# jiaxi98/cnf_ot

Measured on AMD Instinct MI355X. Metric: MC samples/sec through flow fwd+log|detJ| at dim=2, batch=65536, higher is better.
Workload: dtype f32; 1 GPU; configs[1]: OT free dim=2, batch=65536, sample_and_log_prob (RQS fwd + log|detJ|), L=2 H=16 M=2 K=5, params N(0,0.20^2) seed 42; ONE STEP = one evaluator-shaped pass of 10000 time-slices x 65536 samples (cnf_ot/utils.py:311-340), each slice its own condition t, one cnf_sample_logprob call per rank; batch=65536, dim=2, parallelism=slice-shard x1 (contiguous blocks of the step's slices; no collective)

## Files before the change

### cnf_ot_amd/csrc/cnf_common.h

```cpp
#pragma once
#include <mutex>
#include <map>
#include <tuple>
#include <unordered_map>
#include <vector>

#include "cnf_device.h"
#include "cnf_terms.h"
#include "../../include/cnf_ot_amd.h"

namespace cnf {

constexpr int TILE = 256;

struct ModelArgs {
  const float* prep;
  const float* wq;
  int64_t per_layer;
  int64_t per_layer_q;
  int32_t D, L, M;
  SplineConsts sc;
  SplineConstsT<double> scd;
  const double* tabd;
  const double* e2tab;
};

template <class R> __device__ __forceinline__ const SplineConstsT<R>& sc_of(const ModelArgs& a);
template <> __device__ __forceinline__ const SplineConstsT<float>& sc_of<float>(const ModelArgs& a) { return a.sc; }
template <> __device__ __forceinline__ const SplineConstsT<double>& sc_of<double>(const ModelArgs& a) { return a.scd; }
template <class R> __device__ __forceinline__ const R* table_of(const ModelArgs& a);
template <> __device__ __forceinline__ const float* table_of<float>(const ModelArgs& a) { return a.prep; }
template <> __device__ __forceinline__ const double* table_of<double>(const ModelArgs& a) { return a.tabd; }

}

struct CnfModel {
  CnfConfig cfg;
  cnf::SplineConsts sc;
  cnf::SplineConstsT<double> scd;
  int64_t tabd_off;
  int64_t e2_off;
  int precise;
  float* prep;
  int64_t n_params;
  int64_t per_layer;
  int device;
  int num_cus;
  int fast_math;
  int force_spl;
  int use_mfma;
  uint32_t div_magic;
  int64_t per_layer_q;
  int64_t mfma_off;
  int params_set;
  float* grad_slabs;
  int64_t grad_max_blocks;
  int use_pwl;
  int use_dpar;
  float* pwl_stats;
  struct PwlWorkspace { float* tables; int64_t sets; uint32_t epoch; std::vector<float*> retired; };
  std::mutex pwl_mu;
  std::unordered_map<void*, PwlWorkspace> pwl_ws;
  hipEvent_t prep_event;
  void* prep_stream;
  int last_path;
  struct ProfRec { hipEvent_t e0, e1, e2; int64_t samples; int path; };
  int profiling;
  std::vector<ProfRec> prof;
};

enum CnfPath {
  CNF_PATH_NONE = 0,
  CNF_PATH_MLP1 = 1,
  CNF_PATH_MLP2 = 2,
  CNF_PATH_MFMA = 3,
  CNF_PATH_TABLES = 4,
  CNF_PATH_LOSS_MLP = 5,
  CNF_PATH_LOSS_TABLES = 6,
  CNF_PATH_F64 = 7,
  CNF_PATH_DPAR = 9,
  CNF_PATH_DETECT = 8,
  CNF_PATH_FIELDS = 10,
};

static inline bool pwl_network(const CnfConfig& g) {
  return g.dim == 2 && g.hidden_size == 16 && g.num_bins == 5 && g.mlp_num_layers == 2 && !g.periodized;
}
static inline bool pwl_backward_network(const CnfConfig& g) { return pwl_network(g) && g.num_layers <= 4; }
static inline bool pwl_config_ok(const CnfModel* m) { return m->use_pwl && m->fast_math && pwl_network(m->cfg); }
static inline bool pwl_backward_ok(const CnfModel* m) {
  return pwl_config_ok(m) && pwl_backward_network(m->cfg) && m->pwl_stats != nullptr;
}
constexpr int64_t PWL_MIN_SLICE = 8192, PWL_MIN_POINTS = 262144;
static inline bool pwl_term_on_tables(const CnfModel* m, int64_t slice_len, int64_t n_points, bool with_grad) {
  if (with_grad ? !pwl_backward_ok(m) : !pwl_config_ok(m)) return false;
  return m->use_pwl != 1 || (slice_len >= PWL_MIN_SLICE && n_points >= PWL_MIN_POINTS);
}

#ifdef CNF_MINIMAL_CONFIGS
#define CNF_KERNEL_CONFIGS(X) X(16, 5)
#else
#define CNF_KERNEL_CONFIGS(X) \
  X(8, 5) X(16, 4) X(16, 5) X(16, 8) X(16, 10) X(32, 5) X(32, 8) X(64, 5)
#endif

template <class K>
static inline bool ensure_lds(K kernel, size_t bytes) {
  if (bytes > 160 * 1024) return false;
  if (bytes <= 64 * 1024) return true;
  static std::mutex mu;
  static std::map<std::pair<const void*, int>, bool> done;
  int dev = 0;
  if (hipGetDevice(&dev) != hipSuccess) return false;
// ... 85 lines not shown
```

### cnf_ot_amd/csrc/cnf_flow.hip

```cpp
#include "cnf_common.h"
#include <cstdlib>
#include "cnf_pwl_build.h"

#include <math.h>
#include <new>
#include <stdlib.h>
#include <string.h>

namespace cnf {


enum CMode { C_SINGLE = 0, C_PER_SAMPLE = 1, C_TILE_UNIFORM = 2, C_GENERIC = 3 };
enum AuxMode { AUX_LOGDET = 0, AUX_LOGPROB = 1 };


template <class R> struct FlowArgsT {
  ModelArgs m;
  const R* in;
  const R* c;
  R* out;
  R* aux;
  int64_t B;
  int64_t c_block;
  int32_t c_mode, aux_mode;
// ... 1218 lines not shown
  if (!config_valid(cfg)) return CNF_ERR_INVALID;
  if (!cnf_config_supported(cfg)) return CNF_ERR_UNSUPPORTED;
  CnfModel* m = new (std::nothrow) CnfModel();
  if (!m) return CNF_ERR_NOMEM;
  m->cfg = *cfg;
  const int K = cfg->num_bins, P = 3 * K + 1;
  m->n_params = cnf_param_count(cfg);
  m->per_layer = 0;
  for (int d = 1; d < cfg->dim; ++d)
    m->per_layer += cond_floats_p(d, cfg->hidden_size, cfg->mlp_num_layers, P, cfg->periodized != 0);
  m->sc.lo = cfg->range_min; m->sc.hi = cfg->range_max;
  m->sc.min_bin = cfg->min_bin_size; m->sc.min_slope = cfg->min_knot_slope;
  m->sc.span_eff = (float)(((double)cfg->range_max - (double)cfg->range_min) - (double)K * (double)cfg->min_bin_size);
  m->sc.sp_offset = (float)log(exp(1.0 - (double)cfg->min_knot_slope) - 1.0);
  m->fast_math = 1;
  if (hipGetDevice(&m->device) != hipSuccess) { delete m; return CNF_ERR_HIP; }
  hipDeviceProp_t prop;
  if (hipGetDeviceProperties(&prop, m->device) != hipSuccess) { delete m; return CNF_ERR_HIP; }
  m->num_cus = prop.multiProcessorCount;
  m->use_mfma = 2;
  m->use_pwl = 1;
  m->use_dpar = 1;
  m->div_magic = cfg->dim == 1 ? 0u : (uint32_t)((((uint64_t)1 << 32) + (uint64_t)cfg->dim - 1) / (uint64_t)cfg->dim);
  m->per_layer_q = 0; m->mfma_off = 0;
  size_t q_floats = 0;
  if (cfg->hidden_size == 16 && P == 16 && cfg->dim > 1 && !cfg->periodized) {
    for (int d = 1; d < cfg->dim; ++d) m->per_layer_q += cond_floats_mfma(d, cfg->mlp_num_layers);
    m->mfma_off = (hdr_floats(K) + (m->n_params - P) + 3) & ~(int64_t)3;
    q_floats = (size_t)m->per_layer_q * cfg->num_layers;
  }
  m->tabd_off = (hdr_floats(K) + (m->n_params - P) + 4 + (int64_t)q_floats + 1) & ~(int64_t)1;
  m->e2_off = m->tabd_off + 2 * hdr_floats(K);
  m->precise = 1;
  const size_t bytes = (size_t)(m->e2_off + 2 * cnf::EXP2_N) * sizeof(float) + 64;
  m->scd.lo = (double)cfg->range_min; m->scd.hi = (double)cfg->range_max;
  m->scd.min_bin = (double)cfg->min_bin_size; m->scd.min_slope = (double)cfg->min_knot_slope;
  m->scd.span_eff = (m->scd.hi - m->scd.lo) - (double)K * m->scd.min_bin;
  m->scd.sp_offset = log(exp(1.0 - m->scd.min_slope) - 1.0);
  if (hipMalloc((void**)&m->prep, bytes) != hipSuccess) { delete m; return CNF_ERR_NOMEM; }
  {
    double e2[cnf::EXP2_N];
    for (int i = 0; i < cnf::EXP2_N; ++i) e2[i] = exp2(-(double)i / (double)cnf::EXP2_STEPS);
    if (hipMemcpy(m->prep + m->e2_off, e2, sizeof(e2), hipMemcpyHostToDevice) != hipSuccess) {
      (void)hipFree(m->prep); delete m; return CNF_ERR_HIP;
    }
  }
  if (hipEventCreateWithFlags(&m->prep_event, hipEventDisableTiming) != hipSuccess) {
    (void)hipFree(m->prep); delete m; return CNF_ERR_HIP;
  }
  *out = m;
  return CNF_OK;
}

static void prof_clear(CnfModel* m) {
  for (auto& r : m->prof) {
    if (r.e0) (void)hipEventDestroy(r.e0);
    if (r.e1) (void)hipEventDestroy(r.e1);
    if (r.e2) (void)hipEventDestroy(r.e2);
  }
  m->prof.clear();
}

extern "C" void cnf_model_destroy(CnfModel* m) {
  if (!m) return;
  if (m->prep) (void)hipFree(m->prep);
  if (m->grad_slabs) (void)hipFree(m->grad_slabs);
  if (m->pwl_stats) (void)hipFree(m->pwl_stats);
  for (auto& kv : m->pwl_ws) {
    if (kv.second.tables) (void)hipFree(kv.second.tables);
    for (float* p : kv.second.retired) (void)hipFree(p);
  }
  if (m->prep_event) (void)hipEventDestroy(m->prep_event);
  prof_clear(m);
  delete m;
}

extern "C" int cnf_model_last_path(const CnfModel* m) { return m ? m->last_path : CNF_ERR_INVALID; }

extern "C" int cnf_model_set_profiling(CnfModel* m, int on) {
  if (!m) return CNF_ERR_INVALID;
  m->profiling = on ? 1 : 0;
  if (!on) prof_clear(m);
  return CNF_OK;
}

extern "C" int cnf_model_read_profile(CnfModel* m, double* flow_ms, double* build_ms, int64_t* launches,
                                      int64_t* samples) {
  if (!m) return CNF_ERR_INVALID;
  double f = 0.0, b = 0.0;
  int64_t n = 0, smp = 0;
  for (auto& r : m->prof) {
    if (hipEventSynchronize(r.e2) != hipSuccess) return CNF_ERR_HIP;
    float ms = 0.f;
    if (r.e0) { if (hipEventElapsedTime(&ms, r.e0, r.e1) != hipSuccess) return CNF_ERR_HIP; b += ms; }
    if (hipEventElapsedTime(&ms, r.e1, r.e2) != hipSuccess) return CNF_ERR_HIP;
    f += ms; ++n; smp += r.samples;
  }
  prof_clear(m);
  if (flow_ms) *flow_ms = f;
  if (build_ms) *build_ms = b;
  if (launches) *launches = n;
  if (samples) *samples = smp;
  return CNF_OK;
}

struct ProfScope {
  CnfModel* m; hipStream_t s; CnfModel::ProfRec r; bool on;
  ProfScope(CnfModel* m_, hipStream_t s_, bool with_build, int64_t samples, int path) : m(m_), s(s_), on(false) {
    r.e0 = r.e1 = r.e2 = nullptr; r.samples = samples; r.path = path;
    if (!m->profiling || m->prof.size() >= 4096) return;
    if (hipEventCreate(&r.e1) != hipSuccess || hipEventCreate(&r.e2) != hipSuccess) return;
    if (with_build) { if (hipEventCreate(&r.e0) != hipSuccess) return; (void)hipEventRecord(r.e0, s); }
    else (void)hipEventRecord(r.e1, s);
    on = true;
  }
  void built() { if (on && r.e0) (void)hipEventRecord(r.e1, s); }
  void done() { if (on) { (void)hipEventRecord(r.e2, s); m->prof.push_back(r); on = false; } }
};

extern "C" int cnf_model_set_fast_math(CnfModel* m, int on) {
  if (!m) return CNF_ERR_INVALID;
  m->fast_math = on ? 1 : 0;
  return CNF_OK;
// ... 116 lines not shown
    if (!a.gate) m->last_path = CNF_PATH_MLP1;
#define X(HH, KK)                                                                             \
    if (m->cfg.hidden_size == HH && m->cfg.num_bins == KK) {                                  \
      CNF_LAUNCH((flow_kernel<HH, KK, TO_BASE, true, float, false, false, true>), grid1, lds1, stream, a);  \
      return hipGetLastError() == hipSuccess ? CNF_OK : CNF_ERR_HIP;                          \
    }
    CNF_KERNEL_CONFIGS(X)
#undef X
    return CNF_ERR_UNSUPPORTED;
  }
  const bool precise = PR && m->precise;
  const size_t lds = (size_t)(hdr_floats(m->cfg.num_bins) + 2 * a.m.D * ts) * sizeof(float) +
                     (precise ? precise_lds_bytes(m->cfg.num_bins) + sizeof(float) * a.m.D * ts : 0);
  const bool small = a.B <= (int64_t)m->num_cus * 4 * 64 * CNF_MFMA_SMALL_WAVES;
  if (m->fast_math && (m->use_mfma == 1 || (m->use_mfma == 2 && small)) && m->mfma_off > 0 &&
      m->cfg.hidden_size == 16 && m->cfg.num_bins == 5) {
    if (!a.gate) m->last_path = CNF_PATH_MFMA;
    ProfScope ps(m, stream, false, a.B, CNF_PATH_MFMA);
    const bool d2 = m->cfg.dim == 2 && spl == 1;
    if (precise) {
      if (spl == 2) CNF_LAUNCH((flow_kernel<16, 5, TO_BASE, true, v2f, true, PR>), grid, lds, stream, a);
      else if (d2) CNF_LAUNCH((flow_kernel<16, 5, TO_BASE, true, float, true, PR, false, 2>), grid, lds, stream, a);
      else CNF_LAUNCH((flow_kernel<16, 5, TO_BASE, true, float, true, PR>), grid, lds, stream, a);
    } else {
      if (spl == 2) CNF_LAUNCH((flow_kernel<16, 5, TO_BASE, true, v2f, true>), grid, lds, stream, a);
      else if (d2) CNF_LAUNCH((flow_kernel<16, 5, TO_BASE, true, float, true, false, false, 2>), grid, lds, stream, a);
      else CNF_LAUNCH((flow_kernel<16, 5, TO_BASE, true, float, true>), grid, lds, stream, a);
    }
    ps.done();
    return hipGetLastError() == hipSuccess ? CNF_OK : CNF_ERR_HIP;
  }
  if (!a.gate) m->last_path = spl == 2 ? CNF_PATH_MLP2 : CNF_PATH_MLP1;
  ProfScope ps(m, stream, false, a.B, spl == 2 ? CNF_PATH_MLP2 : CNF_PATH_MLP1);
#define X(HH, KK)                                                                             \
  if (m->cfg.hidden_size == HH && m->cfg.num_bins == KK) {                                    \
    if (precise) {                                                                            \
      if (!m->fast_math) CNF_LAUNCH((flow_kernel<HH, KK, TO_BASE, false, float, false, PR>), grid, lds, stream, a);  \
      else if (spl == 2) CNF_LAUNCH((flow_kernel<HH, KK, TO_BASE, true, v2f, false, PR>), grid, lds, stream, a);     \
      else CNF_LAUNCH((flow_kernel<HH, KK, TO_BASE, true, float, false, PR>), grid, lds, stream, a);                 \
    } else {                                                                                  \
      if (!m->fast_math) CNF_LAUNCH((flow_kernel<HH, KK, TO_BASE, false, float>), grid, lds, stream, a);      \
      else if (spl == 2) CNF_LAUNCH((flow_kernel<HH, KK, TO_BASE, true, v2f>), grid, lds, stream, a);         \
      else CNF_LAUNCH((flow_kernel<HH, KK, TO_BASE, true, float>), grid, lds, stream, a);                     \
    }                                                                                         \
    ps.done();                                                                                \
    return hipGetLastError() == hipSuccess ? CNF_OK : CNF_ERR_HIP;                            \
  }
  CNF_KERNEL_CONFIGS(X)
#undef X
  return CNF_ERR_UNSUPPORTED;
}

static void pwl_workspace(CnfModel* m, hipStream_t stream, float** tables, int64_t* sets, uint32_t** flag = nullptr,
                          uint32_t* epoch = nullptr) {
  std::lock_guard<std::mutex> lock(m->pwl_mu);
  auto it = m->pwl_ws.find((void*)stream);
  if (it == m->pwl_ws.end()) { *tables = nullptr; *sets = 0; return; }
  *tables = it->second.tables; *sets = it->second.sets;
  if (flag) { *flag = reinterpret_cast<uint32_t*>(it->second.tables + it->second.sets * m->cfg.num_layers * (int64_t)cnf::PWL_TBL);
              *epoch = ++it->second.epoch; }
}

extern "C" int64_t cnf_model_table_bytes(const CnfModel* m) {
  return m ? (int64_t)sizeof(float) * m->cfg.num_layers * cnf::PWL_TBL : 0;
}

extern "C" int cnf_model_reserve(CnfModel* m, void* stream, int64_t n_sets) {
  if (!m || n_sets < 0) return CNF_ERR_INVALID;
  std::lock_guard<std::mutex> lock(m->pwl_mu);
  CnfModel::PwlWorkspace& ws = m->pwl_ws[stream];
  if (ws.sets >= n_sets && n_sets > 0) return CNF_OK;
  if (ws.tables && n_sets > 0) {
    ws.retired.push_back(ws.tables);
    ws.tables = nullptr; ws.sets = 0;
  }
  if (n_sets == 0) {
    if (hipStreamSynchronize((hipStream_t)stream) != hipSuccess) return CNF_ERR_HIP;
    if (ws.tables) (void)hipFree(ws.tables);
    for (float* p : ws.retired) (void)hipFree(p);
    m->pwl_ws.erase(stream);
    return CNF_OK;
  }
  if (hipMalloc((void**)&ws.tables, (size_t)cnf_model_table_bytes(m) * (size_t)n_sets + 64) != hipSuccess) {
    ws.tables = nullptr; ws.sets = 0;
    return CNF_ERR_NOMEM;
  }
  if (hipMemset(reinterpret_cast<char*>(ws.tables) + (size_t)cnf_model_table_bytes(m) * (size_t)n_sets, 0, 64) != hipSuccess) {
    (void)hipFree(ws.tables); ws.tables = nullptr; ws.sets = 0;
    return CNF_ERR_HIP;
  }
  ws.sets = n_sets; ws.epoch = 0;
  return CNF_OK;
}

extern "C" int64_t cnf_model_reserved(CnfModel* m, void* stream) {
  if (!m) return CNF_ERR_INVALID;
  float* t; int64_t sets;
  pwl_workspace(m, (hipStream_t)stream, &t, &sets);
  return sets;
}

static const int64_t PWL_MAX_SLICES = 2048;

static_assert(cnf::PWL_H == 16, "pwl_network (cnf_common.h) states the tables' network");

extern "C" int cnf_model_has_tables(const CnfModel* m) { return m && pwl_network(m->cfg) ? 1 : 0; }

extern "C" int cnf_model_term_on_tables(const CnfModel* m, int64_t slice_len, int64_t n_points, int with_grad) {
  return m && pwl_term_on_tables(m, slice_len, n_points, with_grad != 0) ? 1 : 0;
}

struct NoiseSrc { uint64_t seed; int64_t first_sample, slice_stride; };

static int run_flow_pwl(CnfModel* m, bool to_base, const float* in, const float* c, int64_t c_block,
                        float* out, float* aux, int aux_mode, int64_t B, hipStream_t stream,
                        bool detect = false, const uint32_t** gate = nullptr, uint32_t* gate_epoch = nullptr,
                        const NoiseSrc* noise = nullptr, const float* built = nullptr, bool in_shared = false) {
  if (!pwl_config_ok(m)) return CNF_ERR_UNSUPPORTED;
  const int L = m->cfg.num_layers;
  const bool precise = to_base && m->precise;
  auto lds_for = [&](int lrows) {
    return (size_t)(((cnf::hdr_floats(5) + 3) & ~3) + L * cnf::pwl_ltbl(lrows)) * sizeof(float) +
           (precise ? precise_lds_bytes(5) : 0);
  };
  const bool full = lds_for(cnf::PWL_NPIECE) <= 160 * 1024;
  size_t lds = lds_for(full ? cnf::PWL_NPIECE : cnf::PWL_LROWS);
  if (lds > 160 * 1024) return CNF_ERR_UNSUPPORTED;
  const int64_t slice_len = c_block < B ? c_block : B;
  const int64_t n_slices = (B + slice_len - 1) / slice_len;
  if (n_slices > 1 && (slice_len & 1)) return CNF_ERR_UNSUPPORTED;
  if ((reinterpret_cast<uintptr_t>(in) & 15) || (reinterpret_cast<uintptr_t>(out) & 15) ||
      (reinterpret_cast<uintptr_t>(aux) & 7))
    return CNF_ERR_UNSUPPORTED;
  const int pwl_threads = cnf::PWL_MAX_THREADS;
  const size_t pwl_min_lds = 82 * 1024;
  const int64_t PWL_TS = 2 * pwl_threads;
  const int64_t tps = (slice_len + PWL_TS - 1) / PWL_TS;
  const int64_t total = n_slices * tps;
  if (total > (1 << 30)) return CNF_ERR_UNSUPPORTED;
  if (m->use_pwl == 1 && (total < 2 * (int64_t)m->num_cus || slice_len < 4 * PWL_TS)) return CNF_ERR_UNSUPPORTED;
  if (pwl_min_lds > lds) lds = pwl_min_lds;
  typedef void (*PwlKernel)(const cnf::PwlArgs);
  constexpr int ALL = cnf::PWL_NPIECE, WIN = cnf::PWL_LROWS;
  const bool l2 = full && L == 2;
  const PwlKernel kern =
      precise ? (l2 ? (PwlKernel)cnf::flow_pwl_kernel<5, true, true, true, ALL, 2>
                    : full ? (PwlKernel)cnf::flow_pwl_kernel<5, true, true, true, ALL> : (PwlKernel)cnf::flow_pwl_kernel<5, true, true, true, WIN>)
      : to_base ? (l2 ? (PwlKernel)cnf::flow_pwl_kernel<5, true, true, false, ALL, 2>
                      : full ? (PwlKernel)cnf::flow_pwl_kernel<5, true, true, false, ALL> : (PwlKernel)cnf::flow_pwl_kernel<5, true, true, false, WIN>)
      : noise ? (l2 ? (PwlKernel)cnf::flow_pwl_kernel<5, false, true, false, ALL, 2, true>
                    : full ? (PwlKernel)cnf::flow_pwl_kernel<5, false, true, false, ALL, 0, true> : (PwlKernel)cnf::flow_pwl_kernel<5, false, true, false, WIN, 0, true>)
                : (l2 ? (PwlKernel)cnf::flow_pwl_kernel<5, false, true, false, ALL, 2>
                      : full ? (PwlKernel)cnf::flow_pwl_kernel<5, false, true, false, ALL> : (PwlKernel)cnf::flow_pwl_kernel<5, false, true, false, WIN>);
  if (!ensure_lds(kern, lds)) return CNF_ERR_UNSUPPORTED;
  int64_t chunk = n_slices < PWL_MAX_SLICES ? n_slices : PWL_MAX_SLICES;
  float* tables = nullptr;
  {
    int64_t sets = 0;
    pwl_workspace(m, stream, &tables, &sets);
    if (sets < chunk) chunk = sets;
    if (chunk < 1 || (built && (chunk < n_slices || built != tables))) return CNF_ERR_UNSUPPORTED;
    if (m->use_pwl == 1 && chunk < n_slices && chunk * tps < (int64_t)m->num_cus) return CNF_ERR_UNSUPPORTED;
  }
  uint32_t* flag = nullptr;
  uint32_t epoch = 0;
  if (detect) {
    int64_t sets = 0;
    pwl_workspace(m, stream, &tables, &sets, &flag, &epoch);
    int64_t g = (B + 4095) / 4096;
    if (g > 4 * (int64_t)m->num_cus) g = 4 * (int64_t)m->num_cus;
    hipLaunchKernelGGL(cnf::cond_uniform_kernel, dim3((unsigned)g), dim3(256), 0, stream, c, B, flag, epoch);
    *gate = flag; *gate_epoch = epoch;
  }
  const double sp_offset = log(exp(1.0 - (double)m->cfg.min_knot_slope) - 1.0);
  m->last_path = detect ? CNF_PATH_DETECT : CNF_PATH_TABLES;
  for (int64_t s0 = 0; s0 < n_slices; s0 += chunk) {
    const int64_t ns = n_slices - s0 < chunk ? n_slices - s0 : chunk;
    const int64_t first = s0 * slice_len;
    ProfScope ps(m, stream, true, (B - first) < ns * slice_len ? (B - first) : ns * slice_len, CNF_PATH_TABLES);
    if (!built)
      hipLaunchKernelGGL(cnf::pwl_build_kernel, dim3((unsigned)(ns * L)), dim3(512), 0, stream,
                         (const float*)(m->prep + cnf::hdr_floats(5)), m->per_layer, c + s0, 0.0f, L, sp_offset, tables);
    ps.built();
    cnf::PwlArgs a;
    a.m = model_args(m);
    a.in_shared = in_shared ? 1 : 0;
    a.in = in ? in + (in_shared ? 0 : first * 2) : nullptr; a.out = out ? out + first * 2 : nullptr; a.aux = aux ? aux + first : nullptr;
    a.seed = noise ? noise->seed : 0; a.slice_stride = noise ? noise->slice_stride : 0;
    a.first_sample = noise ? noise->first_sample + s0 * noise->slice_stride : 0;
    a.tables = tables;
    a.B = (B - first) < ns * slice_len ? (B - first) : ns * slice_len;
    a.slice_len = slice_len;
    a.n_slices = (int32_t)ns; a.tiles_per_slice = (int32_t)tps; a.aux_mode = aux_mode;
    a.gate = flag; a.gate_epoch = epoch; a.gate_want = 0;
    const int64_t tiles = ns * tps;
    const int64_t want = (int64_t)m->num_cus;
    const int64_t grid = tiles < want ? tiles : want;
    hipLaunchKernelGGL(kern, dim3((unsigned)grid), dim3(pwl_threads), lds, stream, a);
    ps.done();
  }
  return hipGetLastError() == hipSuccess ? CNF_OK : CNF_ERR_HIP;
}

int cnf_internal_flow_shared(CnfModel* m, hipStream_t stream, const float* in, const float* c, int64_t slice_len,
                             int64_t n_slices, const float* tables, float* out) {
  return run_flow_pwl(m, false, in, c, slice_len, out, nullptr, 0, n_slices * slice_len, stream, false, nullptr, nullptr,
                      nullptr, tables, true);
}

int cnf_internal_build_tables(CnfModel* m, hipStream_t stream, const float* c, int64_t n, float** tables) {
  if (!pwl_config_ok(m) || n < 1) return CNF_ERR_UNSUPPORTED;
  int64_t sets = 0;
  pwl_workspace(m, stream, tables, &sets);
  if (sets < n) return CNF_ERR_UNSUPPORTED;
  const int L = m->cfg.num_layers;
  const double sp_offset = log(exp(1.0 - (double)m->cfg.min_knot_slope) - 1.0);
  hipLaunchKernelGGL(cnf::pwl_build_kernel, dim3((unsigned)(n * L)), dim3(512), 0, stream,
                     (const float*)(m->prep + cnf::hdr_floats(5)), m->per_layer, c, 0.0f, L, sp_offset, *tables);
  return hipGetLastError() == hipSuccess ? CNF_OK : CNF_ERR_HIP;
}

static int run_flow(CnfModel* m, bool to_base, const float* in, const float* c, int64_t c_block,
                    float* out, float* aux, int aux_mode, int64_t B, void* stream, const NoiseSrc* noise = nullptr) {
  if (!m || (!in && !noise) || (in && noise) || !c || B < 0 || c_block < 1) return CNF_ERR_INVALID;
  if (noise && (to_base || noise->first_sample < 0 || noise->slice_stride < 0)) return CNF_ERR_INVALID;
  if (noise && c_block == 1 && B > 1 && noise->slice_stride != 1) return CNF_ERR_INVALID;
  if (!out && !aux) return CNF_ERR_INVALID;
  if (!m->params_set) return CNF_ERR_INVALID;
  if (B == 0) return CNF_OK;
  if (wait_for_params(m, (hipStream_t)stream) != CNF_OK) return CNF_ERR_HIP;
  const uint32_t* gate = nullptr;
  uint32_t gate_epoch = 0;
  if (c_block == 1 && B > 1) {
    const int r = run_flow_pwl(m, to_base, in, c, B, out, aux, aux_mode, B, (hipStream_t)stream, true, &gate, &gate_epoch, noise);
    if (r != CNF_OK && r != CNF_ERR_UNSUPPORTED) return r;
  } else {
    const int r = run_flow_pwl(m, to_base, in, c, c_block, out, aux, aux_mode, B, (hipStream_t)stream, false, nullptr, nullptr, noise);
    if (r != CNF_ERR_UNSUPPORTED) return r;
  }
  FlowArgs a;
  a.m = model_args(m);
  a.in = in; a.c = c; a.out = out; a.aux = aux;
  a.B = B; a.c_block = c_block;
  a.gate = gate; a.gate_epoch = gate_epoch; a.gate_want = 1;
  a.fd2 = 0; a.fd_h = 0.f; a.fd_inv_dx = 0.f;
  a.seed = noise ? noise->seed : 0; a.first_sample = noise ? noise->first_sample : 0; a.slice_stride = noise ? noise->slice_stride : 0;
  a.aux_mode = aux_mode;
  a.div_magic = m->div_magic;
  int spl = m->fast_math ? samples_per_lane(m, B) : 1;
  if (spl == 2 && (size_t)(hdr_floats(m->cfg.num_bins) + 3 * a.m.D * TILE * 2) * sizeof(float) +
                      precise_lds_bytes(m->cfg.num_bins) > 160 * 1024) spl = 1;
  if (c_block >= B) a.c_mode = C_SINGLE;
  else if (c_block == 1) a.c_mode = C_PER_SAMPLE;
  else if (c_block % (TILE * spl) == 0) a.c_mode = C_TILE_UNIFORM;
  else a.c_mode = C_GENERIC;
  if (!to_base) {
    const int r = launch_flow_dpar(m, a, (hipStream_t)stream);
    if (r != CNF_ERR_UNSUPPORTED) return r;
  }
  return to_base ? launch_flow<true>(m, a, spl, (hipStream_t)stream)
                 : launch_flow<false>(m, a, spl, (hipStream_t)stream);
}

extern "C" int cnf_forward_logdet(CnfModel* m, const float* x, const float* c, int64_t c_block,
                                  float* y, float* logdet, int64_t B, void* stream) {
  return run_flow(m, false, x, c, c_block, y, logdet, AUX_LOGDET, B, stream);
}

extern "C" int cnf_inverse_logdet(CnfModel* m, const float* y, const float* c, int64_t c_block,
                                  float* x, float* logdet, int64_t B, void* stream) {
// ... 127 lines not shown
  if (!state || n < 0 || (n > 0 && !out)) return CNF_ERR_INVALID;
  if (n == 0) return CNF_OK;
  int64_t grid = (n + 255) / 256;
  if (grid > 4096) grid = 4096;
  hipLaunchKernelGGL(cnf::fill_uniform_kernel, dim3((unsigned)grid), dim3(256), 0, (hipStream_t)stream, state, first, n, scale, out);
  return hipGetLastError() == hipSuccess ? CNF_OK : CNF_ERR_HIP;
}

extern "C" int cnf_mixture_source_dev(const uint64_t* state, uint64_t first_sample, int64_t n, const float* z, float* out,
                                      int32_t* comp, void* stream) {
  if (!state || n < 0 || (n > 0 && !out && !comp) || (out && !z)) return CNF_ERR_INVALID;
  if (n == 0) return CNF_OK;
  int64_t grid = (n + 255) / 256;
  if (grid > 4096) grid = 4096;
  hipLaunchKernelGGL(cnf::mixture_source_kernel, dim3((unsigned)grid), dim3(256), 0, (hipStream_t)stream, state, first_sample,
                     n, z, out, comp);
  return hipGetLastError() == hipSuccess ? CNF_OK : CNF_ERR_HIP;
}


static int loss_terms_pwl(CnfModel* m, const CnfLossSpec* spec, const float* pts, int64_t slice_stride,
                          uint64_t seed, int64_t first_sample, const float* t, int64_t n_slices, int64_t B,
                          double* sums, hipStream_t stream) {
  if (!pwl_config_ok(m)) return CNF_ERR_UNSUPPORTED;
  const int L = m->cfg.num_layers;
  const int kind = spec->kind;
  const bool kin = kind <= CNF_TERM_FLOW_MATCHING;
  const int n_sets = kind == CNF_TERM_KINETIC ? 2 : (kin ? 3 : 1);
  const int threads = cnf::PWL_MAX_THREADS;
  const int64_t ts = 2 * threads;
  const size_t lds = (size_t)(((cnf::hdr_floats(5) + 3) & ~3) + n_sets * L * cnf::PWL_LTBL + 2 * ts) * sizeof(float);
  if (lds > 160 * 1024) return CNF_ERR_UNSUPPORTED;
  const int64_t tps = (B + ts - 1) / ts;
  const int64_t total = n_slices * tps;
  if (total > (1 << 30)) return CNF_ERR_UNSUPPORTED;
  if (m->use_pwl == 1 && (total < 2 * (int64_t)m->num_cus || B < 4 * ts)) return CNF_ERR_UNSUPPORTED;
  if (!ensure_lds(cnf::loss_pwl_kernel<5, true>, lds)) return CNF_ERR_UNSUPPORTED;
  int64_t chunk = n_slices < PWL_MAX_SLICES ? n_slices : PWL_MAX_SLICES;
  float* tables = nullptr;
  {
    int64_t sets = 0;
    pwl_workspace(m, stream, &tables, &sets);
    if (sets / n_sets < chunk) chunk = sets / n_sets;
    if (chunk < 1) return CNF_ERR_UNSUPPORTED;
    if (m->use_pwl == 1 && chunk < n_slices && chunk * tps < (int64_t)m->num_cus) return CNF_ERR_UNSUPPORTED;
  }
  const double sp_offset = log(exp(1.0 - (double)m->cfg.min_knot_slope) - 1.0);
  m->last_path = CNF_PATH_LOSS_TABLES;
  for (int64_t s0 = 0; s0 < n_slices; s0 += chunk) {
    const int64_t ns = n_slices - s0 < chunk ? n_slices - s0 : chunk;
    const int64_t set_stride = ns * L * (int64_t)cnf::PWL_TBL;
    for (int s = 0; s < n_sets; ++s) {
      const float off = !kin ? 0.0f : (s == 0 ? -0.5f * spec->dt : (s == 1 ? 0.5f * spec->dt : 0.0f));
      hipLaunchKernelGGL(cnf::pwl_build_kernel, dim3((unsigned)(ns * L)), dim3(512), 0, stream,
                         (const float*)(m->prep + cnf::hdr_floats(5)), m->per_layer, t + s0, off, L, sp_offset,
                         tables + s * set_stride);
    }
    cnf::LossPwlArgs a;
    a.m = model_args(m); a.spec = *spec; a.t = t + s0; a.sums = sums + s0; a.tables = tables;
    a.pts = pts ? pts + s0 * slice_stride * 2 : nullptr;
    a.B = B; a.n_slices = ns; a.pts_slice_stride = slice_stride;
    a.seed = seed; a.first_sample = first_sample + s0 * slice_stride;
    a.n_sets = n_sets; a.tiles_per_slice = (int32_t)tps;
    a.mix = cnf::density_mix_consts(*spec, 2);
    const int64_t tiles = ns * tps;
    const int64_t grid = tiles < m->num_cus ? tiles : m->num_cus;
    hipLaunchKernelGGL((cnf::loss_pwl_kernel<5, true>), dim3((unsigned)grid), dim3(threads), lds, stream, a);
  }
  return hipGetLastError() == hipSuccess ? CNF_OK : CNF_ERR_HIP;
}

static int loss_terms_impl(CnfModel* m, const CnfLossSpec* spec, const float* pts, int64_t slice_stride,
                           uint64_t seed, int64_t first_sample, const float* t, int64_t n_slices, int64_t B,
                           double* sums, void* stream_) {
  if (!m || !spec || !t || !sums || n_slices < 0 || B < 0 || slice_stride < 0 || first_sample < 0) return CNF_ERR_INVALID;
  if (!m->params_set) return CNF_ERR_INVALID;
  if (term_spec_check(spec, m->cfg.dim) != CNF_OK) return CNF_ERR_INVALID;
  if (m->cfg.periodized) return CNF_ERR_UNSUPPORTED;
  const int D = m->cfg.dim;
  hipStream_t stream = (hipStream_t)stream_;
  if (n_slices == 0) return CNF_OK;
  if (hipMemsetAsync(sums, 0, sizeof(double) * (size_t)n_slices, stream) != hipSuccess) return CNF_ERR_HIP;
  if (B == 0) return CNF_OK;
  if (wait_for_params(m, stream) != CNF_OK) return CNF_ERR_HIP;
  {
    const int r = loss_terms_pwl(m, spec, pts, slice_stride, seed, first_sample, t, n_slices, B, sums, stream);
    if (r != CNF_ERR_UNSUPPORTED) return r;
  }
  m->last_path = CNF_PATH_LOSS_MLP;

  LossArgs a;
  a.m = model_args(m); a.spec = *spec; a.pts = pts; a.t = t; a.sums = sums;
  a.B = B; a.n_slices = n_slices; a.pts_slice_stride = slice_stride;
  a.div_magic = m->div_magic; a.seed = seed; a.first_sample = first_sample;
  a.mix = density_mix_consts(*spec, D);
  int spl = (m->fast_math && n_slices * B >= (int64_t)m->num_cus * 4 * 64 * 2) ? 2 : 1;
  if (m->force_spl == 1 || m->force_spl == 2) spl = m->fast_math ? m->force_spl : 1;
  if (spl == 2 && (size_t)(5 * D * TILE * 2) * sizeof(float) > 64 * 1024) spl = 1;
  const int64_t ts = (int64_t)TILE * spl;
  const size_t lds = (size_t)(hdr_floats(m->cfg.num_bins) + 5 * D * ts) * sizeof(float);
  if (lds > 160 * 1024) return CNF_ERR_UNSUPPORTED;
  int64_t grid = ((B + ts - 1) / ts) * n_slices;
  const int64_t cap = (int64_t)m->num_cus * 8;
  if (grid > cap) grid = cap;
#define X(HH, KK)                                                                             \
  if (m->cfg.hidden_size == HH && m->cfg.num_bins == KK) {                                    \
    if (!m->fast_math) CNF_LAUNCH((loss_kernel<HH, KK, false, float>), grid, lds, stream, a);                 \
// ... 185 lines not shown
```

### cnf_ot_amd/csrc/cnf_pwl_build.h

```cpp
#pragma once

#include "cnf_pwl.h"

namespace cnf {

__global__ __launch_bounds__(512) void pwl_build_kernel(const float* __restrict__ weights ,
                                                        int64_t per_layer, const float* __restrict__ cvals,
                                                        float c_offset, int L, double sp_offset,
                                                        float* __restrict__ tables) {
  __shared__ double a1[PWL_H], b1v[PWL_H], W1[PWL_H * PWL_H], bb1[PWL_H], Wo[PWL_H * PWL_P], bo[PWL_P];
  __shared__ double bpu[PWL_H], sbp[PWL_H];
  __shared__ double candu[PWL_NPIECE - 1], cand[PWL_NPIECE - 1];
  __shared__ double PQ[PWL_CHUNK * PWL_H * 2];
  __shared__ double RAW[PWL_CHUNK * PWL_P * 2];
  __shared__ int bad[PWL_NPIECE];
  __shared__ double urefs[PWL_CHUNK];
  __shared__ int icnt[17], ioff[17];
  __shared__ double IPQ[17 * PWL_H * 2];
  __shared__ int biv[PWL_NPIECE];
  const int tid = threadIdx.x;
  const int slice = blockIdx.x / L, l = blockIdx.x % L;
  const float* w = weights + l * per_layer;
  const double c = (double)cvals[slice] + (double)c_offset;
  const double INF = __longlong_as_double(0x7ff0000000000000LL);
  if (tid < PWL_H) {
    const double a = (double)w[PWL_H + tid], b = (double)w[tid] * c + (double)w[2 * PWL_H + tid];
    a1[tid] = a;
    b1v[tid] = b;
    bpu[tid] = a != 0.0 ? -b / a : INF;
    bb1[tid] = (double)w[3 * PWL_H + 256 + tid];
    bo[tid] = (double)w[3 * PWL_H + 256 + PWL_H + 256 + tid];
  }
  for (int i = tid; i < 256; i += blockDim.x) {
    W1[i] = (double)w[3 * PWL_H + i];
    Wo[i] = (double)w[3 * PWL_H + 256 + PWL_H + i];
  }
  __syncthreads();
  if (tid < PWL_H) {
    const double v = bpu[tid];
    int r = 0;
    for (int j = 0; j < PWL_H; ++j) r += (bpu[j] < v || (bpu[j] == v && j < tid)) ? 1 : 0;
    sbp[r] = v;
  }
  __syncthreads();
  auto test_point = [&](double lo, double hi) -> double {
    const bool fl = lo > -INF, fh = hi < INF;
    return fl && fh ? 0.5 * (lo + hi) : (fl ? lo + 1.0 : (fh ? hi - 1.0 : 0.0));
  };
  double root = INF;
  const int iv = tid / PWL_H, kk = tid % PWL_H;
  if (tid < 17 * PWL_H) {
    const double lo = iv == 0 ? -INF : sbp[iv - 1], hi = iv == PWL_H ? INF : sbp[iv];
    if (lo < INF) {
      const double u = test_point(lo, hi);
      double P = 0.0, Q = bb1[kk];
      for (int j = 0; j < PWL_H; ++j) {
        const double on = a1[j] * u + b1v[j] > 0.0 ? W1[j * PWL_H + kk] : 0.0;
        P += on * a1[j];
        Q += on * b1v[j];
      }
      IPQ[2 * tid] = P; IPQ[2 * tid + 1] = Q;
      if (lo < hi && P != 0.0) { const double r = -Q / P; if (r > lo && r < hi) root = r; }
    }
    candu[PWL_H + tid] = root;
  }
  for (int p = tid; p < PWL_NPIECE - 1; p += blockDim.x) cand[p] = INF;
  for (int p = tid; p < PWL_NPIECE; p += blockDim.x) bad[p] = 0;
  __syncthreads();
  int rank_in = 0;
  if (tid < 17 * PWL_H) {
    int cnt = 0;
    for (int j = 0; j < PWL_H; ++j) {
      const double o = candu[PWL_H + iv * PWL_H + j];
      rank_in += (o < root || (o == root && j < kk)) ? 1 : 0;
      cnt += o < INF ? 1 : 0;
    }
    if (kk == 0) icnt[iv] = cnt;
  }
  __syncthreads();
  if (tid < 17) {
    int sum = 0;
    for (int i = 0; i < tid; ++i) sum += icnt[i];
    ioff[tid] = sum;
  }
  __syncthreads();
  if (tid < 17 * PWL_H && root < INF) {
    cand[iv + ioff[iv] + rank_in] = root;
    biv[iv + ioff[iv] + rank_in] = iv;
  }
  if (tid < PWL_H && sbp[tid] < INF) {
    cand[tid + ioff[tid] + icnt[tid]] = sbp[tid];
    biv[tid + ioff[tid] + icnt[tid]] = tid;
  }
  int n1 = 0;
  for (int j = 0; j < PWL_H; ++j) n1 += sbp[j] < INF ? 1 : 0;
  const int n = n1 + ioff[16] + icnt[16];
  __syncthreads();
  float* T = tables + (int64_t)blockIdx.x * PWL_TBL;
  for (int p = tid; p < PWL_NBP; p += blockDim.x)
    T[p] = p == PWL_N_SLOT ? __int_as_float(n) : (p < n ? (float)cand[p] : __int_as_float(0x7fc00000));
  const double LOG2E_D = 1.4426950408889634;
  for (int base = 0; base <= n; base += PWL_CHUNK) {
    const int np = n + 1 - base < PWL_CHUNK ? n + 1 - base : PWL_CHUNK;
    for (int t = tid; t < np * PWL_H; t += blockDim.x) {
      const int p = base + (t >> 4), k = t & 15;
      const double lo = p == 0 ? -INF : cand[p - 1], hi = p < n ? cand[p] : INF;
      const double u = test_point(lo, hi);
      const int ivp = p < n ? biv[p] : n1;
      const double P = IPQ[2 * (ivp * PWL_H + k)], Q = IPQ[2 * (ivp * PWL_H + k) + 1];
      const bool act = P * u + Q > 0.0;
      PQ[2 * t] = act ? P : 0.0;
      PQ[2 * t + 1] = act ? Q : 0.0;
    }
    __syncthreads();
    for (int t = tid; t < np * PWL_P; t += blockDim.x) {
      const int pl = t >> 4, m = t & 15, p = base + pl;
      double S = 0.0, Tt = bo[m];
      for (int k = 0; k < PWL_H; ++k) {
        const double wo = Wo[k * PWL_P + m];
        S += wo * PQ[2 * (pl * PWL_H + k)];
        Tt += wo * PQ[2 * (pl * PWL_H + k) + 1];
      }
      const double lo = p == 0 ? -INF : cand[p - 1], hi = p < n ? cand[p] : INF;
      const double nearest = lo > 0.0 ? lo : (hi < 0.0 ? hi : 0.0);
      const float uref = (float)(nearest < (double)PWL_GMIN ? (double)PWL_GMIN : (nearest > -(double)PWL_GMIN ? -(double)PWL_GMIN : nearest));
      Tt += S * (double)uref;
      if (m == 0) {
        T[PWL_OFF_REF + p] = uref; urefs[pl] = (double)uref;
        T[PWL_OFF_PIECE + p * PWL_ROW + 2 * PWL_P] = uref;
      }
      RAW[2 * t] = S;
      RAW[2 * t + 1] = Tt;
    }
    __syncthreads();
    for (int t = tid; t < np * PWL_P; t += blockDim.x) {
      const int pl = t >> 4, m = t & 15, p = base + pl;
      double S = RAW[2 * t], Tt = RAW[2 * t + 1];
      const double lo = p == 0 ? -INF : cand[p - 1], hi = p < n ? cand[p] : INF;
      const double uref = urefs[pl];
      const double ulo = fmax(lo, (double)PWL_GMIN - 0.01), uhi = fmin(hi, -(double)PWL_GMIN + 0.01);
      bool out_of_bounds = false;
      if (m < 2 * 5) {
        const int r0 = m < 5 ? 0 : 5;
        const double uc = ulo <= uhi ? 0.5 * (ulo + uhi) : uref;
        double Mc = -INF, Mlo = -INF, Mhi = -INF;
        for (int k = r0; k < r0 + 5; ++k) {
          const double Sk = RAW[2 * (pl * PWL_P + k)], Tk = RAW[2 * (pl * PWL_P + k) + 1];
          Mc = fmax(Mc, Tk + Sk * (uc - uref));
          Mlo = fmax(Mlo, Tk + Sk * (ulo - uref));
          Mhi = fmax(Mhi, Tk + Sk * (uhi - uref));
        }
        if (ulo <= uhi)
          out_of_bounds = fmax(fabs(Mlo - Mc), fabs(Mhi - Mc)) * LOG2E_D > PWL_FAST_LOGIT;
        S *= LOG2E_D;
        Tt = (Tt - Mc) * LOG2E_D;
      } else {
        Tt += sp_offset;
        if (ulo <= uhi) {
          const double a = Tt + S * (ulo - uref), b = Tt + S * (uhi - uref);
          out_of_bounds = fmin(a, b) < PWL_FAST_SLOPE_LO || fmax(a, b) > PWL_FAST_SLOPE_HI;
        }
        S *= LOG2E_D; Tt *= LOG2E_D;
      }
      if (out_of_bounds || !(S == S) || !(Tt == Tt)) bad[p] = 1;
      float* row = T + PWL_OFF_PIECE + p * PWL_ROW;
      row[m] = (float)S;
      row[PWL_P + m] = (float)Tt;
    }
    __syncthreads();
  }
  int* delta = reinterpret_cast<int*>(PQ);
  static_assert(sizeof(double) * PWL_CHUNK * PWL_H * 2 >= sizeof(int) * (PWL_NG + 16), "scratch for the grid scan");
  constexpr int CPT = 4;
  static_assert(PWL_NG == 512 * CPT, "one thread owns four consecutive cells (512 threads)");
  for (int g = tid; g < PWL_NG + 16; g += blockDim.x) delta[g] = 0;
  __syncthreads();
  for (int p = tid; p < n; p += blockDim.x) {
    const double gb = ceil((cand[p] + 1e-4 - (double)PWL_GMIN) * (double)PWL_GSCALE);
    const int g0 = gb < 1.0 ? 1 : (gb >= (double)PWL_NG ? PWL_NG : (int)gb);
    atomicAdd(&delta[g0], 1);
  }
  __syncthreads();
  {
    const int g0 = tid * CPT;
    int c0 = delta[g0], c1 = c0 + delta[g0 + 1], c2 = c1 + delta[g0 + 2], c3 = c2 + delta[g0 + 3];
    int run = c3;
#pragma unroll
    for (int off = 1; off < 64; off <<= 1) {
      const int v = __shfl_up(run, off, 64);
      if ((tid & 63) >= off) run += v;
    }
    int* wtot = delta + PWL_NG + 8;
    __syncthreads();
    if ((tid & 63) == 63) wtot[tid >> 6] = run;
    __syncthreads();
    int before = run - c3;
    for (int w2 = 0; w2 < (tid >> 6); ++w2) before += wtot[w2];
    const int cnt[CPT] = {before + c0, before + c1, before + c2, before + c3};
#pragma unroll
    for (int i = 0; i < CPT; ++i) {
      const int g = g0 + i;
      const int lo_ = g == 0 ? 0 : cnt[i];
      const double xr = g == PWL_NG - 1 ? INF : (double)PWL_GMIN + (double)(g + 1) / (double)PWL_GSCALE + 1e-4;
      int mark = (g == 0 || g == PWL_NG - 1) ? 1 : 0;
      for (int p = lo_; p <= n && !mark; ++p) {
        mark |= bad[p];
        if (p < n && cand[p] > xr) break;
      }
      const bool many = lo_ + 2 < n && cand[lo_ + 2] <= xr;
      reinterpret_cast<uint16_t*>(T + PWL_OFF_GRID)[g] =
          (uint16_t)((uint32_t)lo_ | (mark ? PWL_G_GENERAL : 0u) | (many ? PWL_G_MANY : 0u));
    }
  }
}


}
```

Before: 88.91 billion samples/s.

## Double-buffer PWL table builds on a side stream to overlap evaluation

When the slice count exceeds the table workspace, the workspace is split into two halves. The table build for the next chunk is launched on a non-blocking side stream, and events order it against the evaluation of the current chunk, so building and evaluating can overlap. The builder kernel is templated on block size, with a 256-thread variant with a different unroll factor for the side stream. Halving the chunk doubles the number of launches and adds event waits. The overlap only pays off if the builder and the evaluator can actually share CUs.

```diff
diff --git a/cnf_ot_amd/csrc/cnf_common.h b/cnf_ot_amd/csrc/cnf_common.h
--- a/cnf_ot_amd/csrc/cnf_common.h
+++ b/cnf_ot_amd/csrc/cnf_common.h
@@ -58,7 +58,8 @@
   int use_pwl;
   int use_dpar;
   float* pwl_stats;
-  struct PwlWorkspace { float* tables; int64_t sets; uint32_t epoch; std::vector<float*> retired; };
+  struct PwlPipe { hipStream_t side; hipEvent_t fork, built[2], read[2]; };
+  struct PwlWorkspace { float* tables; int64_t sets; uint32_t epoch; std::vector<float*> retired; PwlPipe pipe; };
   std::mutex pwl_mu;
   std::unordered_map<void*, PwlWorkspace> pwl_ws;
   hipEvent_t prep_event;
diff --git a/cnf_ot_amd/csrc/cnf_flow.hip b/cnf_ot_amd/csrc/cnf_flow.hip
--- a/cnf_ot_amd/csrc/cnf_flow.hip
+++ b/cnf_ot_amd/csrc/cnf_flow.hip
@@ -1294,6 +1294,26 @@
   return CNF_OK;
 }
 
+static void pwl_pipe_destroy(CnfModel::PwlPipe& p) {
+  if (p.side) (void)hipStreamDestroy(p.side);
+  if (p.fork) (void)hipEventDestroy(p.fork);
+  for (int h = 0; h < 2; ++h) {
+    if (p.built[h]) (void)hipEventDestroy(p.built[h]);
+    if (p.read[h]) (void)hipEventDestroy(p.read[h]);
+  }
+  p = CnfModel::PwlPipe{};
+}
+
+static void pwl_pipe_create(CnfModel::PwlPipe& p) {
+  if (p.side) return;
+  bool ok = hipStreamCreateWithFlags(&p.side, hipStreamNonBlocking) == hipSuccess &&
+            hipEventCreateWithFlags(&p.fork, hipEventDisableTiming) == hipSuccess;
+  for (int h = 0; h < 2 && ok; ++h)
+    ok = hipEventCreateWithFlags(&p.built[h], hipEventDisableTiming) == hipSuccess &&
+         hipEventCreateWithFlags(&p.read[h], hipEventDisableTiming) == hipSuccess;
+  if (!ok) { (void)hipGetLastError(); pwl_pipe_destroy(p); }
+}
+
 static void prof_clear(CnfModel* m) {
   for (auto& r : m->prof) {
     if (r.e0) (void)hipEventDestroy(r.e0);
@@ -1311,6 +1331,7 @@
   for (auto& kv : m->pwl_ws) {
     if (kv.second.tables) (void)hipFree(kv.second.tables);
     for (float* p : kv.second.retired) (void)hipFree(p);
+    pwl_pipe_destroy(kv.second.pipe);
   }
   if (m->prep_event) (void)hipEventDestroy(m->prep_event);
   prof_clear(m);
@@ -1533,9 +1554,10 @@
 }
 
 static void pwl_workspace(CnfModel* m, hipStream_t stream, float** tables, int64_t* sets, uint32_t** flag = nullptr,
-                          uint32_t* epoch = nullptr) {
+                          uint32_t* epoch = nullptr, CnfModel::PwlPipe* pipe = nullptr) {
   std::lock_guard<std::mutex> lock(m->pwl_mu);
   auto it = m->pwl_ws.find((void*)stream);
+  if (pipe) *pipe = it == m->pwl_ws.end() ? CnfModel::PwlPipe{} : it->second.pipe;
   if (it == m->pwl_ws.end()) { *tables = nullptr; *sets = 0; return; }
   *tables = it->second.tables; *sets = it->second.sets;
   if (flag) { *flag = reinterpret_cast<uint32_t*>(it->second.tables + it->second.sets * m->cfg.num_layers * (int64_t)cnf::PWL_TBL);
@@ -1559,6 +1581,7 @@
     if (hipStreamSynchronize((hipStream_t)stream) != hipSuccess) return CNF_ERR_HIP;
     if (ws.tables) (void)hipFree(ws.tables);
     for (float* p : ws.retired) (void)hipFree(p);
+    pwl_pipe_destroy(ws.pipe);
     m->pwl_ws.erase(stream);
     return CNF_OK;
   }
@@ -1571,6 +1594,7 @@
     return CNF_ERR_HIP;
   }
   ws.sets = n_sets; ws.epoch = 0;
+  pwl_pipe_create(ws.pipe);
   return CNF_OK;
 }
 
@@ -1636,12 +1660,23 @@
   if (!ensure_lds(kern, lds)) return CNF_ERR_UNSUPPORTED;
   int64_t chunk = n_slices < PWL_MAX_SLICES ? n_slices : PWL_MAX_SLICES;
   float* tables = nullptr;
+  CnfModel::PwlPipe pipe{};
+  bool pipelined = false;
   {
     int64_t sets = 0;
-    pwl_workspace(m, stream, &tables, &sets);
+    pwl_workspace(m, stream, &tables, &sets, nullptr, nullptr, &pipe);
     if (sets < chunk) chunk = sets;
     if (chunk < 1 || (built && (chunk < n_slices || built != tables))) return CNF_ERR_UNSUPPORTED;
     if (m->use_pwl == 1 && chunk < n_slices && chunk * tps < (int64_t)m->num_cus) return CNF_ERR_UNSUPPORTED;
+    if (!built && n_slices > sets && sets >= 2 && pipe.side && !m->profiling) {
+      const int64_t half = sets / 2 < PWL_MAX_SLICES ? sets / 2 : PWL_MAX_SLICES;
+      hipStreamCaptureStatus cap = hipStreamCaptureStatusNone;
+      if (hipStreamIsCapturing(stream, &cap) != hipSuccess) { (void)hipGetLastError(); cap = hipStreamCaptureStatusActive; }
+      if (cap == hipStreamCaptureStatusNone && (m->use_pwl != 1 || half * tps >= (int64_t)m->num_cus)) {
+        pipelined = true;
+        chunk = half;
+      }
+    }
   }
   uint32_t* flag = nullptr;
   uint32_t epoch = 0;
@@ -1655,13 +1690,35 @@
   }
   const double sp_offset = log(exp(1.0 - (double)m->cfg.min_knot_slope) - 1.0);
   m->last_path = detect ? CNF_PATH_DETECT : CNF_PATH_TABLES;
-  for (int64_t s0 = 0; s0 < n_slices; s0 += chunk) {
+  const float* weights = (const float*)(m->prep + cnf::hdr_floats(5));
+  if (pipelined) {
+    if (hipEventRecord(pipe.fork, stream) != hipSuccess || hipStreamWaitEvent(pipe.side, pipe.fork, 0) != hipSuccess)
+      return CNF_ERR_HIP;
+  }
+  auto build_ahead = [&](int64_t s0, int h) -> bool {
+    const int64_t ns = n_slices - s0 < chunk ? n_slices - s0 : chunk;
+    if (hipStreamWaitEvent(pipe.side, pipe.read[h], 0) != hipSuccess) return false;
+    hipLaunchKernelGGL(cnf::pwl_build_kernel<cnf::PWL_BUILD_SIDE>, dim3((unsigned)(ns * L)), dim3(cnf::PWL_BUILD_SIDE), 0,
+                       pipe.side, weights, m->per_layer, c + s0, 0.0f, L, sp_offset,
+                       tables + (int64_t)h * chunk * L * cnf::PWL_TBL);
+    return hipEventRecord(pipe.built[h], pipe.side) == hipSuccess;
+  };
+  int64_t k = 0;
+  for (int64_t s0 = 0; s0 < n_slices; s0 += chunk, ++k) {
     const int64_t ns = n_slices - s0 < chunk ? n_slices - s0 : chunk;
     const int64_t first = s0 * slice_len;
+    const int h = pipelined ? (int)(k & 1) : 0;
+    float* const chunk_tables = tables + (int64_t)h * chunk * L * cnf::PWL_TBL;
     ProfScope ps(m, stream, true, (B - first) < ns * slice_len ? (B - first) : ns * slice_len, CNF_PATH_TABLES);
-    if (!built)
-      hipLaunchKernelGGL(cnf::pwl_build_kernel, dim3((unsigned)(ns * L)), dim3(512), 0, stream,
-                         (const float*)(m->prep + cnf::hdr_floats(5)), m->per_layer, c + s0, 0.0f, L, sp_offset, tables);
+    if (pipelined) {
+      if (k == 0)
+        hipLaunchKernelGGL(cnf::pwl_build_kernel<512>, dim3((unsigned)(ns * L)), dim3(512), 0, stream,
+                           weights, m->per_layer, c + s0, 0.0f, L, sp_offset, chunk_tables);
+      else if (hipStreamWaitEvent(stream, pipe.built[h], 0) != hipSuccess) return CNF_ERR_HIP;
+      if (s0 + chunk < n_slices && !build_ahead(s0 + chunk, h ^ 1)) return CNF_ERR_HIP;
+    } else if (!built)
+      hipLaunchKernelGGL(cnf::pwl_build_kernel<512>, dim3((unsigned)(ns * L)), dim3(512), 0, stream,
+                         weights, m->per_layer, c + s0, 0.0f, L, sp_offset, chunk_tables);
     ps.built();
     cnf::PwlArgs a;
     a.m = model_args(m);
@@ -1669,7 +1726,7 @@
     a.in = in ? in + (in_shared ? 0 : first * 2) : nullptr; a.out = out ? out + first * 2 : nullptr; a.aux = aux ? aux + first : nullptr;
     a.seed = noise ? noise->seed : 0; a.slice_stride = noise ? noise->slice_stride : 0;
     a.first_sample = noise ? noise->first_sample + s0 * noise->slice_stride : 0;
-    a.tables = tables;
+    a.tables = chunk_tables;
     a.B = (B - first) < ns * slice_len ? (B - first) : ns * slice_len;
     a.slice_len = slice_len;
     a.n_slices = (int32_t)ns; a.tiles_per_slice = (int32_t)tps; a.aux_mode = aux_mode;
@@ -1678,6 +1735,7 @@
     const int64_t want = (int64_t)m->num_cus;
     const int64_t grid = tiles < want ? tiles : want;
     hipLaunchKernelGGL(kern, dim3((unsigned)grid), dim3(pwl_threads), lds, stream, a);
+    if (pipelined && hipEventRecord(pipe.read[h], stream) != hipSuccess) return CNF_ERR_HIP;
     ps.done();
   }
   return hipGetLastError() == hipSuccess ? CNF_OK : CNF_ERR_HIP;
@@ -1696,7 +1754,7 @@
   if (sets < n) return CNF_ERR_UNSUPPORTED;
   const int L = m->cfg.num_layers;
   const double sp_offset = log(exp(1.0 - (double)m->cfg.min_knot_slope) - 1.0);
-  hipLaunchKernelGGL(cnf::pwl_build_kernel, dim3((unsigned)(n * L)), dim3(512), 0, stream,
+  hipLaunchKernelGGL(cnf::pwl_build_kernel<512>, dim3((unsigned)(n * L)), dim3(512), 0, stream,
                      (const float*)(m->prep + cnf::hdr_floats(5)), m->per_layer, c, 0.0f, L, sp_offset, *tables);
   return hipGetLastError() == hipSuccess ? CNF_OK : CNF_ERR_HIP;
 }
@@ -1930,7 +1988,7 @@
     const int64_t set_stride = ns * L * (int64_t)cnf::PWL_TBL;
     for (int s = 0; s < n_sets; ++s) {
       const float off = !kin ? 0.0f : (s == 0 ? -0.5f * spec->dt : (s == 1 ? 0.5f * spec->dt : 0.0f));
-      hipLaunchKernelGGL(cnf::pwl_build_kernel, dim3((unsigned)(ns * L)), dim3(512), 0, stream,
+      hipLaunchKernelGGL(cnf::pwl_build_kernel<512>, dim3((unsigned)(ns * L)), dim3(512), 0, stream,
                          (const float*)(m->prep + cnf::hdr_floats(5)), m->per_layer, t + s0, off, L, sp_offset,
                          tables + s * set_stride);
     }
diff --git a/cnf_ot_amd/csrc/cnf_pwl_build.h b/cnf_ot_amd/csrc/cnf_pwl_build.h
--- a/cnf_ot_amd/csrc/cnf_pwl_build.h
+++ b/cnf_ot_amd/csrc/cnf_pwl_build.h
@@ -4,10 +4,15 @@
 
 namespace cnf {
 
-__global__ __launch_bounds__(512) void pwl_build_kernel(const float* __restrict__ weights ,
-                                                        int64_t per_layer, const float* __restrict__ cvals,
-                                                        float c_offset, int L, double sp_offset,
-                                                        float* __restrict__ tables) {
+constexpr int PWL_BUILD_SIDE = 256;
+constexpr int PWL_BUILD_SIDE_UNROLL = 8;
+
+template <int NT, int UNR>
+__device__ __forceinline__ void pwl_build_body(const float* __restrict__ weights ,
+                                               int64_t per_layer, const float* __restrict__ cvals,
+                                               float c_offset, int L, double sp_offset,
+                                               float* __restrict__ tables) {
+  static_assert(NT == 512 || NT == 256, "block shapes of the builder");
   __shared__ double a1[PWL_H], b1v[PWL_H], W1[PWL_H * PWL_H], bb1[PWL_H], Wo[PWL_H * PWL_P], bo[PWL_P];
   __shared__ double bpu[PWL_H], sbp[PWL_H];
   __shared__ double candu[PWL_NPIECE - 1], cand[PWL_NPIECE - 1];
@@ -47,35 +52,47 @@
     const bool fl = lo > -INF, fh = hi < INF;
     return fl && fh ? 0.5 * (lo + hi) : (fl ? lo + 1.0 : (fh ? hi - 1.0 : 0.0));
   };
-  double root = INF;
-  const int iv = tid / PWL_H, kk = tid % PWL_H;
-  if (tid < 17 * PWL_H) {
-    const double lo = iv == 0 ? -INF : sbp[iv - 1], hi = iv == PWL_H ? INF : sbp[iv];
-    if (lo < INF) {
-      const double u = test_point(lo, hi);
-      double P = 0.0, Q = bb1[kk];
-      for (int j = 0; j < PWL_H; ++j) {
-        const double on = a1[j] * u + b1v[j] > 0.0 ? W1[j * PWL_H + kk] : 0.0;
-        P += on * a1[j];
-        Q += on * b1v[j];
-      }
-      IPQ[2 * tid] = P; IPQ[2 * tid + 1] = Q;
-      if (lo < hi && P != 0.0) { const double r = -Q / P; if (r > lo && r < hi) root = r; }
-    }
-    candu[PWL_H + tid] = root;
+  constexpr int NTASK = 17 * PWL_H, TPT = (NTASK + NT - 1) / NT;
+  double root[TPT];
+#pragma unroll
+  for (int r = 0; r < TPT; ++r) {
+    root[r] = INF;
+    const int task = tid + r * NT, iv = task / PWL_H, kk = task % PWL_H;
+    if (task < NTASK) {
+      const double lo = iv == 0 ? -INF : sbp[iv - 1], hi = iv == PWL_H ? INF : sbp[iv];
+      if (lo < INF) {
+        const double u = test_point(lo, hi);
+        double P = 0.0, Q = bb1[kk];
+#pragma unroll UNR
+        for (int j = 0; j < PWL_H; ++j) {
+          const double on = a1[j] * u + b1v[j] > 0.0 ? W1[j * PWL_H + kk] : 0.0;
+          P += on * a1[j];
+          Q += on * b1v[j];
+        }
+        IPQ[2 * task] = P; IPQ[2 * task + 1] = Q;
+        if (lo < hi && P != 0.0) { const double rt = -Q / P; if (rt > lo && rt < hi) root[r] = rt; }
+      }
+      candu[PWL_H + task] = root[r];
+    }
   }
   for (int p = tid; p < PWL_NPIECE - 1; p += blockDim.x) cand[p] = INF;
   for (int p = tid; p < PWL_NPIECE; p += blockDim.x) bad[p] = 0;
   __syncthreads();
-  int rank_in = 0;
-  if (tid < 17 * PWL_H) {
-    int cnt = 0;
-    for (int j = 0; j < PWL_H; ++j) {
-      const double o = candu[PWL_H + iv * PWL_H + j];
-      rank_in += (o < root || (o == root && j < kk)) ? 1 : 0;
-      cnt += o < INF ? 1 : 0;
-    }
-    if (kk == 0) icnt[iv] = cnt;
+  int rank_in[TPT];
+#pragma unroll
+  for (int r = 0; r < TPT; ++r) {
+    rank_in[r] = 0;
+    const int task = tid + r * NT, iv = task / PWL_H, kk = task % PWL_H;
+    if (task < NTASK) {
+      int cnt = 0;
+#pragma unroll UNR
+      for (int j = 0; j < PWL_H; ++j) {
+        const double o = candu[PWL_H + iv * PWL_H + j];
+        rank_in[r] += (o < root[r] || (o == root[r] && j < kk)) ? 1 : 0;
+        cnt += o < INF ? 1 : 0;
+      }
+      if (kk == 0) icnt[iv] = cnt;
+    }
   }
   __syncthreads();
   if (tid < 17) {
@@ -84,9 +101,13 @@
     ioff[tid] = sum;
   }
   __syncthreads();
-  if (tid < 17 * PWL_H && root < INF) {
-    cand[iv + ioff[iv] + rank_in] = root;
-    biv[iv + ioff[iv] + rank_in] = iv;
+#pragma unroll
+  for (int r = 0; r < TPT; ++r) {
+    const int task = tid + r * NT, iv = task / PWL_H;
+    if (task < NTASK && root[r] < INF) {
+      cand[iv + ioff[iv] + rank_in[r]] = root[r];
+      biv[iv + ioff[iv] + rank_in[r]] = iv;
+    }
   }
   if (tid < PWL_H && sbp[tid] < INF) {
     cand[tid + ioff[tid] + icnt[tid]] = sbp[tid];
@@ -116,6 +137,7 @@
     for (int t = tid; t < np * PWL_P; t += blockDim.x) {
       const int pl = t >> 4, m = t & 15, p = base + pl;
       double S = 0.0, Tt = bo[m];
+#pragma unroll UNR
       for (int k = 0; k < PWL_H; ++k) {
         const double wo = Wo[k * PWL_P + m];
         S += wo * PQ[2 * (pl * PWL_H + k)];
@@ -144,6 +166,7 @@
         const int r0 = m < 5 ? 0 : 5;
         const double uc = ulo <= uhi ? 0.5 * (ulo + uhi) : uref;
         double Mc = -INF, Mlo = -INF, Mhi = -INF;
+#pragma unroll UNR
         for (int k = r0; k < r0 + 5; ++k) {
           const double Sk = RAW[2 * (pl * PWL_P + k)], Tk = RAW[2 * (pl * PWL_P + k) + 1];
           Mc = fmax(Mc, Tk + Sk * (uc - uref));
@@ -171,8 +194,8 @@
   }
   int* delta = reinterpret_cast<int*>(PQ);
   static_assert(sizeof(double) * PWL_CHUNK * PWL_H * 2 >= sizeof(int) * (PWL_NG + 16), "scratch for the grid scan");
-  constexpr int CPT = 4;
-  static_assert(PWL_NG == 512 * CPT, "one thread owns four consecutive cells (512 threads)");
+  constexpr int CPT = PWL_NG / NT, NWAVE = NT / 64;
+  static_assert(PWL_NG == NT * CPT && NWAVE <= 8, "one thread owns CPT consecutive cells; eight slots for wave totals");
   for (int g = tid; g < PWL_NG + 16; g += blockDim.x) delta[g] = 0;
   __syncthreads();
   for (int p = tid; p < n; p += blockDim.x) {
@@ -183,8 +206,11 @@
   __syncthreads();
   {
     const int g0 = tid * CPT;
-    int c0 = delta[g0], c1 = c0 + delta[g0 + 1], c2 = c1 + delta[g0 + 2], c3 = c2 + delta[g0 + 3];
-    int run = c3;
+    int cs[CPT];
+    cs[0] = delta[g0];
+#pragma unroll
+    for (int i = 1; i < CPT; ++i) cs[i] = cs[i - 1] + delta[g0 + i];
+    int run = cs[CPT - 1];
 #pragma unroll
     for (int off = 1; off < 64; off <<= 1) {
       const int v = __shfl_up(run, off, 64);
@@ -194,13 +220,12 @@
     __syncthreads();
     if ((tid & 63) == 63) wtot[tid >> 6] = run;
     __syncthreads();
-    int before = run - c3;
+    int before = run - cs[CPT - 1];
     for (int w2 = 0; w2 < (tid >> 6); ++w2) before += wtot[w2];
-    const int cnt[CPT] = {before + c0, before + c1, before + c2, before + c3};
 #pragma unroll
     for (int i = 0; i < CPT; ++i) {
       const int g = g0 + i;
-      const int lo_ = g == 0 ? 0 : cnt[i];
+      const int lo_ = g == 0 ? 0 : before + cs[i];
       const double xr = g == PWL_NG - 1 ? INF : (double)PWL_GMIN + (double)(g + 1) / (double)PWL_GSCALE + 1e-4;
       int mark = (g == 0 || g == PWL_NG - 1) ? 1 : 0;
       for (int p = lo_; p <= n && !mark; ++p) {
@@ -214,5 +239,23 @@
   }
 }
 
-
-}
+template <int NT>
+__global__ void pwl_build_kernel(const float* __restrict__ weights, int64_t per_layer, const float* __restrict__ cvals,
+                                 float c_offset, int L, double sp_offset, float* __restrict__ tables);
+
+template <>
+__global__ __launch_bounds__(512) void pwl_build_kernel<512>(const float* __restrict__ weights, int64_t per_layer,
+                                                             const float* __restrict__ cvals, float c_offset, int L,
+                                                             double sp_offset, float* __restrict__ tables) {
+  pwl_build_body<512, PWL_H>(weights, per_layer, cvals, c_offset, L, sp_offset, tables);
+}
+
+template <>
+__global__ __launch_bounds__(PWL_BUILD_SIDE)
+void pwl_build_kernel<PWL_BUILD_SIDE>(const float* __restrict__ weights, int64_t per_layer,
+                                      const float* __restrict__ cvals, float c_offset, int L, double sp_offset,
+                                      float* __restrict__ tables) {
+  pwl_build_body<PWL_BUILD_SIDE, PWL_BUILD_SIDE_UNROLL>(weights, per_layer, cvals, c_offset, L, sp_offset, tables);
+}
+
+}
```

Measured after the change: 78.38 billion samples/s. 0.882x the previous value.
